# SandraLouise/SVJedi-graph

Measured on AMD Instinct MI355X. Metric: GAF alignments classified/sec (classify + count all-reduce + genotype, text resident in HBM), higher is better.
Workload: dtype u8/int64 (classify), f64 (likelihood)

## Files before the change

svjedi-graph_amd/csrc/svjg_capi.hip:

```cpp
#include "svjg_kernels.h"
#include "svjg_host_tables.h"
#include "svjg_pass.h"
#include <rccl/rccl.h>
#include <errno.h>
#include <math.h>
#include <stdio.h>
#include <stdlib.h>
#include <string.h>
#include <fcntl.h>
#include <unistd.h>
#include <string>
#include <thread>
#include <vector>

using namespace svjg;
typedef struct svjg_ctx svjg_ctx;

static thread_local std::string g_init_error;

#include <memory>
#include <mutex>
namespace {
struct TablesCache {
    std::mutex mu;
// ... 18 lines not shown
    h = fold64(g.chrom_names, (size_t)g.chrom_off[g.n_chrom], h);
    const uint64_t tail[3] = {g.d_over, g.flags, g.n_slots};
    return fold64(tail, sizeof tail, h);
}

std::shared_ptr<const KernelTables> kernel_tables_for(const svjg_graph &g) {
    const uint64_t key[6] = {g.n_nodes, g.n_edges, g.n_hits, g.n_chrom, graph_digest(g, 1), graph_digest(g, 0xD6E8FEB86659FD93ull)};
    std::lock_guard<std::mutex> lk(g_tables.mu);
    if (!g_tables.kt || memcmp(key, g_tables.key, sizeof key) != 0) {
        g_tables.kt = std::make_shared<const KernelTables>(build_kernel_tables(g));
        memcpy(g_tables.key, key, sizeof key);
    }
    return g_tables.kt;
}
}

extern "C" void svjg_release_host_tables(void) {
    std::lock_guard<std::mutex> lk(g_tables.mu);
    g_tables.kt.reset();
    memset(g_tables.key, 0, sizeof g_tables.key);
}

constexpr int STAGE_THREADS = 4;
constexpr uint64_t STAGE_PIECE = 8ull << 20;

constexpr int RUN_SLOTS = 3;

struct svjg_ctx {
    int device = 0;
    int wall_khz = 0;
    int n_cu = 256;
    int occ_main = 0;
    hipStream_t stream = nullptr, copy_stream = nullptr;
    hipEvent_t ev[6] = {};
    std::string err;
    bool have_graph = false, have_counts = false;
    svjg_node *d_nodes = nullptr;  svjg_edge *d_edges = nullptr;  uint32_t *d_hits = nullptr;
    uint8_t *d_cnames = nullptr;   uint32_t *d_coff = nullptr, *d_clo = nullptr, *d_chash = nullptr, *d_names = nullptr, *d_links = nullptr, *d_nok = nullptr;  uint16_t *d_disp = nullptr;  uint32_t *d_ihits = nullptr, *d_pfx = nullptr;
    GraphView gv{};
    uint32_t names_len = 0, gflags = 0, n_slots = 0;
    unsigned long long *d_counts = nullptr, *d_snap = nullptr;
    uint8_t *d_gaf = nullptr;  uint64_t gaf_cap = 0, gaf_bytes = 0;  bool have_gaf = false;
    char *h_stage[STAGE_THREADS * 2] = {};
    hipStream_t stage_stream[STAGE_THREADS] = {};
    hipEvent_t stage_ev[STAGE_THREADS * 2] = {};
    uint64_t *d_deferred = nullptr;  uint64_t deferred_cap = 0;
    svjg_hitrec *d_recs = nullptr;   uint64_t rec_cap = 0;
    uint64_t *d_host = nullptr;      uint64_t host_cap = 0;
    DevStatus *d_st = nullptr;
    unsigned long long *d_dbg = nullptr;
    uint32_t *d_long = nullptr;
    DevStatus *h_stp = nullptr;
    DevStatus &hs() { return *h_stp; }
    uint64_t total_deferred = 0;
    dd *d_logfact = nullptr;  uint32_t logfact_n = 0;  dd *d_bsum = nullptr;
    unsigned int *d_maxn = nullptr;
    void *d_rows = nullptr;  uint64_t rows_cap = 0;
    void *h_rows = nullptr;  uint64_t h_rows_cap = 0;
    uint64_t geno_rows = 0;
    struct RunSlot {
        void *d = nullptr;  uint64_t d_cap = 0;  void *h = nullptr;  uint64_t h_cap = 0;  void *h_dev = nullptr;
        unsigned long long *counts = nullptr;  uint64_t counts_cap = 0;
        hipEvent_t ev[6] = {};  hipEvent_t computed = nullptr, copied = nullptr;
        uint64_t base_offset = 0;  uint32_t min_support = 0;  double err = 0;  bool had_text = false, slow_end_own = false, timed_by_events = false;
        bool clean = false;
    } run[RUN_SLOTS];
    int run_head = 0, run_tail = 0, run_inflight = 0;
    int counts_in_slot = -1;
    void *d_run_in = nullptr;  uint64_t d_run_in_cap = 0;  uint64_t run_rows = 0;  bool have_rows = false;
    float ms_main = 0, ms_slow = 0, ms_geno = 0;
    float ms_main_stamps = 0, ms_main_events = 0;
    ncclComm_t comm = nullptr;
    bool allreduce_second = false;
    uint64_t part_total = 0, part_need = 0, part_next = 0;
};

#define HIPCHK(ctx, call)                                                                         \
    do {                                                                                          \
        hipError_t e_ = (call);                                                                   \
        if (e_ != hipSuccess) {                                                                   \
            (ctx)->err = std::string(#call) + ": " + hipGetErrorString(e_);                       \
            return SVJG_E_HIP;                                                                    \
        }                                                                                         \
    } while (0)

extern "C" int svjg_abi_version(void) { return SVJG_ABI_VERSION; }

extern "C" int svjg_device_count(void) {
    int n = 0;
    if (hipGetDeviceCount(&n) != hipSuccess) return 0;
    return n;
}

extern "C" const char *svjg_last_error(const svjg_ctx *ctx) { return ctx ? ctx->err.c_str() : g_init_error.c_str(); }

extern "C" int svjg_init(int device, svjg_ctx **out) {
    if (!out) return SVJG_E_ARG;
    *out = nullptr;
    int n = 0;
    hipError_t e = hipGetDeviceCount(&n);
    if (e != hipSuccess || n <= 0) {
        g_init_error = "no HIP device visible (libsvjg_hip has no CPU fallback)";
        return SVJG_E_NO_DEVICE;
    }
    if (device < 0 || device >= n) { g_init_error = "device index out of range"; return SVJG_E_ARG; }
    svjg_ctx *c = new svjg_ctx();
// ... 21 lines not shown
}

static void free_graph(svjg_ctx *c) {
    hipFree(c->d_nodes); hipFree(c->d_edges); hipFree(c->d_hits); hipFree(c->d_cnames); hipFree(c->d_coff);
    hipFree(c->d_clo); hipFree(c->d_chash); hipFree(c->d_counts); hipFree(c->d_snap); hipFree(c->d_names); hipFree(c->d_links); hipFree(c->d_disp); hipFree(c->d_ihits); hipFree(c->d_nok); hipFree(c->d_pfx);
    c->d_pfx = nullptr; c->d_nok = nullptr; c->d_names = nullptr; c->d_links = nullptr; c->d_disp = nullptr; c->d_ihits = nullptr;
    c->d_nodes = nullptr; c->d_edges = nullptr; c->d_hits = nullptr; c->d_cnames = nullptr; c->d_coff = nullptr;
    c->d_clo = nullptr; c->d_chash = nullptr; c->d_counts = nullptr; c->d_snap = nullptr;
    c->have_graph = false; c->have_counts = false;
    for (auto &r : c->run) r.clean = false;
}

extern "C" void svjg_destroy(svjg_ctx *c) {
    if (!c) return;
    hipSetDevice(c->device);
    if (c->stream) hipStreamSynchronize(c->stream);
    if (c->copy_stream) hipStreamSynchronize(c->copy_stream);
    if (c->comm) ncclCommDestroy(c->comm);
    free_graph(c);
    hipFree(c->d_long);
    hipFree(c->d_gaf); hipFree(c->d_deferred); hipFree(c->d_recs); hipFree(c->d_host); hipFree(c->d_st); hipFree(c->d_logfact);
    hipFree(c->d_bsum); hipFree(c->d_maxn); hipFree(c->d_rows); hipFree(c->d_run_in);
    for (auto &r : c->run) {
        hipFree(r.d); hipFree(r.counts);
        if (r.h) hipHostFree(r.h);
        for (auto &e : r.ev) if (e) hipEventDestroy(e);
        if (r.computed) hipEventDestroy(r.computed);
        if (r.copied) hipEventDestroy(r.copied);
    }
    if (c->h_rows) hipHostFree(c->h_rows);
    if (c->h_stp) hipHostFree(c->h_stp);
    for (auto &b : c->h_stage) if (b) hipHostFree(b);
    for (auto &ev : c->stage_ev) if (ev) hipEventDestroy(ev);
    for (auto &st : c->stage_stream) if (st) hipStreamDestroy(st);
    for (auto &ev : c->ev) if (ev) hipEventDestroy(ev);
    if (c->copy_stream) hipStreamDestroy(c->copy_stream);
    if (c->stream) hipStreamDestroy(c->stream);
    delete c;
}

template <class T>
static int upload(svjg_ctx *c, T **dst, const T *src, uint64_t n, uint64_t extra = 0) {
    HIPCHK(c, hipMalloc((void **)dst, (n + extra + 1) * sizeof(T)));
    if (n) HIPCHK(c, hipMemcpyAsync(*dst, src, n * sizeof(T), hipMemcpyHostToDevice, c->stream));
    return 0;
}

#ifndef SVJG_SMALL_CHUNK
#define SVJG_SMALL_CHUNK 65536
#endif
#ifndef SVJG_FIRST_SHARE
#define SVJG_FIRST_SHARE 0.85
#endif
constexpr uint64_t SMALL_CHUNK = SVJG_SMALL_CHUNK;
constexpr double FIRST_CHUNK_SHARE = SVJG_FIRST_SHARE;

static int reset_status(svjg_ctx *c, bool all) {
    if (all) {
        c->hs() = c->h_stp[1]; c->total_deferred = 0;
        HIPCHK(c, hipMemcpyAsync(c->d_st, &c->h_stp[1], sizeof(DevStatus), hipMemcpyHostToDevice, c->stream));
        return 0;
    }
    c->hs().n_deferred = 0; c->hs().overflow = 0; c->hs().next_chunk = 0;
    HIPCHK(c, hipMemcpyAsync(c->d_st, &c->hs(), sizeof(DevStatus), hipMemcpyHostToDevice, c->stream));
    return 0;
}

extern "C" int svjg_load_graph(svjg_ctx *c, const svjg_graph *g) {
    if (!c || !g || !g->nodes || !g->chrom_off || !g->chrom_node_lo) return SVJG_E_ARG;
    if (g->n_nodes >= 0x7FFFFFFFull || g->n_edges >= 0x7FFFFFFFull || g->n_chrom >= 65535) { c->err = "graph too large"; return SVJG_E_ARG; }
    if (g->d_over >= 0x80000000u) { c->err = "d_over too large"; return SVJG_E_ARG; }
    HIPCHK(c, hipSetDevice(c->device));
    free_graph(c);
    int rc;
    struct Undo { svjg_ctx *c; bool armed = true; ~Undo() { if (armed) { hipStreamSynchronize(c->stream); free_graph(c); } } } undo{c};
    if ((rc = upload(c, &c->d_nodes, g->nodes, g->n_nodes + 1))) return rc;
    if ((rc = upload(c, &c->d_edges, g->edges, g->n_edges))) return rc;
    if ((rc = upload(c, &c->d_hits, g->hits, g->n_hits))) return rc;
    c->names_len = g->chrom_off[g->n_chrom];
    if ((rc = upload(c, &c->d_cnames, (const uint8_t *)g->chrom_names, c->names_len, 8))) return rc;
    if ((rc = upload(c, &c->d_coff, g->chrom_off, g->n_chrom + 1))) return rc;
    if ((rc = upload(c, &c->d_clo, g->chrom_node_lo, g->n_chrom + 1))) return rc;
    std::vector<uint32_t> hash = build_chrom_hash(*g);
    if ((rc = upload(c, &c->d_chash, hash.data(), hash.size()))) return rc;
    const std::shared_ptr<const KernelTables> ktp = kernel_tables_for(*g);
    const KernelTables &kt = *ktp;
    if ((rc = upload(c, &c->d_names, kt.names.data(), kt.names.size()))) return rc;
    if ((rc = upload(c, &c->d_links, kt.links.data(), kt.links.size()))) return rc;
    if ((rc = upload(c, &c->d_disp, kt.disp.data(), kt.disp.size()))) return rc;
    if ((rc = upload(c, &c->d_ihits, kt.ihits.data(), kt.ihits.size()))) return rc;
    if ((rc = upload(c, &c->d_nok, kt.node_of_kid.data(), kt.node_of_kid.size()))) return rc;
    if (!kt.name_pfx.empty() && (rc = upload(c, &c->d_pfx, kt.name_pfx.data(), kt.name_pfx.size()))) return rc;
    HIPCHK(c, hipStreamSynchronize(c->stream));
    c->gv.nodes = c->d_nodes; c->gv.n_nodes = (uint32_t)g->n_nodes; c->gv.edges = c->d_edges; c->gv.hits = c->d_hits;
    c->gv.chrom_names = c->d_cnames; c->gv.chrom_off = c->d_coff; c->gv.chrom_lo = c->d_clo; c->gv.chrom_hash = c->d_chash;
    c->gv.n_chrom = g->n_chrom; c->gv.hash_mask = (uint32_t)hash.size() - 1; c->gv.d_over = g->d_over;
    c->gv.dover_list = (g->flags & SVJG_GRAPH_DOVER_LIST) ? 1u : 0u;
    c->gv.name_pfx = c->d_pfx;
    c->gv.node_of_kid = c->d_nok; c->gv.name_tab = c->d_names; c->gv.name_ihits = c->d_ihits; c->gv.name_disp = c->d_disp; c->gv.name_slots = kt.name_slots; c->gv.name_buckets = kt.name_buckets;
    c->gv.name_complete = (kt.names_left_out == 0 && kt.names_skipped == 0) ? 1u : 0u;
    c->gv.link_tab = c->d_links; c->gv.link_mask = kt.link_mask; c->gv.link_seed = kt.link_seed;
    c->gflags = g->flags;
    if (g->flags & SVJG_GRAPH_DOVER_LIST) c->gflags |= SVJG_GRAPH_ALL_SLOW;
    if (kt.links_left_out) c->gflags |= SVJG_GRAPH_ALL_SLOW;
    c->n_slots = g->n_slots;
    HIPCHK(c, hipMalloc((void **)&c->d_counts, ((uint64_t)g->n_slots + GUARD_WORDS) * 8));
    HIPCHK(c, hipMalloc((void **)&c->d_snap, ((uint64_t)g->n_slots + GUARD_WORDS) * 8));
    c->have_graph = true; c->have_counts = true;
    undo.armed = false;
    return svjg_reset_counts(c);
}

extern "C" int svjg_alloc_counts(svjg_ctx *c, uint32_t n_slots) {
    if (!c) return SVJG_E_ARG;
    HIPCHK(c, hipSetDevice(c->device));
    free_graph(c);
// ... 116 lines not shown
        if (rc) return rc;
    }
    return gaf_finish(c, n, need);
}

static int ensure(svjg_ctx *c, void **p, uint64_t *cap, uint64_t want, size_t elem, bool keep) {
    if (want <= *cap) return 0;
    const uint64_t asked = want;
    if (keep && *cap && want < *cap + *cap / 2) want = *cap + *cap / 2;
    void *q = nullptr;
    if (want != asked && hipMalloc(&q, want * elem) != hipSuccess) { (void)hipGetLastError(); q = nullptr; want = asked; }
    if (!q) HIPCHK(c, hipMalloc(&q, want * elem));
    if (keep && *p && *cap) HIPCHK(c, hipMemcpyAsync(q, *p, *cap * elem, hipMemcpyDeviceToDevice, c->stream));
    HIPCHK(c, hipStreamSynchronize(c->stream));
    hipFree(*p);
    *p = q; *cap = want;
    return 0;
}

static int fetch_slot_counts(svjg_ctx *c) {
    if (c->counts_in_slot < 0) return 0;
    const int k = c->counts_in_slot;
    c->counts_in_slot = -1;
    HIPCHK(c, hipSetDevice(c->device));
    if (c->run[k].copied) HIPCHK(c, hipStreamWaitEvent(c->stream, c->run[k].copied, 0));
    HIPCHK(c, hipMemcpyAsync(c->d_counts, c->run[k].counts, ((uint64_t)c->n_slots + GUARD_WORDS) * 8, hipMemcpyDeviceToDevice, c->stream));
    return 0;
}

static uint64_t deferred_want(const svjg_ctx *c, uint64_t n) { return (c->gflags & SVJG_GRAPH_ALL_SLOW) ? n / 24 + 64 : (n / 4096 + 65536); }

static void main_launch_setup(svjg_ctx *c, uint64_t begin, uint64_t end, uint64_t base_offset, int want_hits, ClassifyArgs &a, uint32_t &grid, size_t &lds) {
    const uint64_t n = end - begin;
    const bool all_slow = (c->gflags & SVJG_GRAPH_ALL_SLOW) != 0;
    a.gaf = c->d_gaf; a.begin = begin; a.n_bytes = end; a.base_offset = base_offset; a.g = c->gv;
    a.all_slow = all_slow; a.want_hits = want_hits != 0;
#ifdef SVJG_ABLATE
    { const char *dg = getenv("SVJG_DIAG"); a.diag = dg ? (uint32_t)atoi(dg) : 0u; }
#endif
    a.counts = c->d_counts; a.deferred = c->d_deferred; a.deferred_cap = c->deferred_cap;
    a.recs = c->d_recs; a.rec_cap = c->rec_cap; a.host_lines = c->d_host; a.host_cap = c->host_cap; a.st = c->d_st; a.dbg = c->d_dbg;
    lds = LDS_MAIN;
    if (c->occ_main < 1) {
        int occ = 0;
        if (hipOccupancyMaxActiveBlocksPerMultiprocessor(&occ, k_classify_main, (int)WG, lds) != hipSuccess || occ < 1) occ = 1;
        const int by_lds = (int)((160u * 1024u) / ((lds + LDS_GRANULE - 1) / LDS_GRANULE * LDS_GRANULE));
        if (by_lds >= 1 && occ > by_lds) occ = by_lds;
        c->occ_main = occ;
        hipFree(c->d_long); c->d_long = nullptr;
#ifdef SVJG_ABLATE
        { const char *oc = getenv("SVJG_OCC"); fprintf(stderr, "[svjg diag] occupancy API: %d workgroups of %u threads per CU (LDS %zu)\n", occ, WG, lds); if (oc && atoi(oc) > 0) c->occ_main = atoi(oc); }
#endif
    }
    const uint64_t full = (uint64_t)c->n_cu * (uint64_t)c->occ_main;
    if (!c->d_long && hipMalloc((void **)&c->d_long, full * LONG_WORDS * sizeof(uint32_t)) != hipSuccess) c->d_long = nullptr;
    a.long_pre = c->d_long;
    const uint64_t share = (n + full - 1) / full;
    uint64_t region = (share + 15) & ~15ull;
    a.small = 0;
    if (share >= 8 * SMALL_CHUNK) { region = ((uint64_t)(share * FIRST_CHUNK_SHARE) + 15) & ~15ull; a.small = SMALL_CHUNK; }
    if (region < TEXT) region = TEXT;
    a.region = region;
    const uint64_t want_grid = (n + region - 1) / region;
    grid = (uint32_t)(want_grid < full ? want_grid : full);
}

constexpr uint64_t EXACT_ROUND_PER_CU = 4;
constexpr uint64_t STEP_WAVE_ROUNDS = 30;
constexpr uint64_t FUSED_WAVE_ROUNDS = 16;
static int launch_exact(svjg_ctx *c, const ClassifyArgs &a, uint64_t wave_rounds, const NextPass &nx) {
    const uint64_t wave_limit = wave_rounds * EXACT_ROUND_PER_CU * (uint64_t)c->n_cu;
    hipLaunchKernelGGL(k_classify_exact, dim3((uint32_t)c->n_cu * EXACT_BLOCKS_PER_CU), dim3(EXACT_TPB), 0, c->stream, a, wave_limit, nx);
    HIPCHK(c, hipGetLastError());
    return 0;
}

static int classify_range(svjg_ctx *c, uint64_t begin, uint64_t end, uint64_t base_offset, int want_hits) {
    HIPCHK(c, hipSetDevice(c->device));
    { const int rc0 = fetch_slot_counts(c); if (rc0) return rc0; }
    if (end <= begin) return 0;
    const uint64_t n = end - begin;
    uint64_t def_want = deferred_want(c, n);
    uint64_t rec_want = want_hits ? c->hs().n_recs + n / 40 + 65536 : 0;
    uint64_t host_want = c->hs().n_host + 4096;
    int rc;
    for (int attempt = 0; attempt < 3; ++attempt) {
        if ((rc = ensure(c, (void **)&c->d_deferred, &c->deferred_cap, def_want, sizeof(uint64_t), false))) return rc;
        if ((rc = ensure(c, (void **)&c->d_host, &c->host_cap, host_want, sizeof(uint64_t), true))) return rc;
        if (want_hits && (rc = ensure(c, (void **)&c->d_recs, &c->rec_cap, rec_want, sizeof(svjg_hitrec), true))) return rc;
        HIPCHK(c, hipMemcpyAsync(c->d_snap, c->d_counts, ((uint64_t)c->n_slots + GUARD_WORDS) * 8, hipMemcpyDeviceToDevice, c->stream));
        DevStatus before = c->hs();
        if ((rc = reset_status(c, false))) return rc;
        ClassifyArgs a{};
        uint32_t grid = 0;
        size_t lds = 0;
        main_launch_setup(c, begin, end, base_offset, want_hits, a, grid, lds);
        if (!a.long_pre) { c->err = "no memory for the workers' scratch words"; return SVJG_E_NOMEM; }
#ifdef SVJG_TIMING
        if (a.diag & 16u) HIPCHK(c, hipMemsetAsync(c->d_dbg, 0, 32 * 8, c->stream));
#endif
        HIPCHK(c, hipEventRecord(c->ev[0], c->stream));
        hipLaunchKernelGGL(k_classify_main, dim3(grid), dim3(WG), lds, c->stream, a);
        HIPCHK(c, hipGetLastError());
        HIPCHK(c, hipEventRecord(c->ev[1], c->stream));
        HIPCHK(c, hipMemcpyAsync(&c->hs(), c->d_st, sizeof(DevStatus), hipMemcpyDeviceToHost, c->stream));
        HIPCHK(c, hipStreamSynchronize(c->stream));
        const uint64_t n_def = c->hs().n_deferred;
#ifdef SVJG_TIMING
        if (a.diag & 16u) {
            unsigned long long d[16];
            HIPCHK(c, hipMemcpy(d, c->d_dbg, sizeof d, hipMemcpyDeviceToHost));
            fprintf(stderr, "[svjg diag] sub-passes of long lines: first sweep counting %llu, first sweep measuring only %llu, second sweep %llu; nodes in sub-passes %llu\n", d[12], d[13], d[14], d[15]);
            fprintf(stderr, "[svjg diag] wave time per phase (sum over waves, counter ticks)  A+B1 %llu  prefix %llu  B2 %llu  R1 %llu  NP: lists %llu  names+disp %llu  records %llu  scan+search %llu  links+atomics %llu  R6+end %llu;  passes %llu (sub-passes of long lines %llu), nodes in them %llu\n",
                    d[0], d[1], d[2], d[3], d[8], d[9], d[4], 0ull, d[6], d[7], d[10], d[11], d[5]);
        }
#endif
        c->ms_slow = 0;
        if (n_def && !(c->hs().overflow & 1u)) {
            HIPCHK(c, hipEventRecord(c->ev[2], c->stream));
            if ((rc = launch_exact(c, a, STEP_WAVE_ROUNDS, NextPass{}))) return rc;
            HIPCHK(c, hipEventRecord(c->ev[3], c->stream));
            HIPCHK(c, hipMemcpyAsync(&c->hs(), c->d_st, sizeof(DevStatus), hipMemcpyDeviceToHost, c->stream));
            HIPCHK(c, hipStreamSynchronize(c->stream));
            HIPCHK(c, hipEventElapsedTime(&c->ms_slow, c->ev[2], c->ev[3]));
#ifdef SVJG_TIMING
            if (a.diag & 16u) {
                unsigned long long d[8];
                HIPCHK(c, hipMemcpy(d, c->d_dbg + 16, sizeof d, hipMemcpyDeviceToHost));
                fprintf(stderr, "[svjg diag] one wave per line, the longest any line took per step (counter ticks): terminator + staging %llu  per-line part %llu  piece table %llu  nodes %llu  links %llu\n",
                        d[0], d[1], d[2], d[3], d[4]);
                unsigned long long l[5];
                HIPCHK(c, hipMemcpy(l, c->d_dbg + 24, sizeof l, hipMemcpyDeviceToHost));
                fprintf(stderr, "[svjg diag] one lane per line, ticks summed over the blocks of 64 lines: terminators + staging %llu  per-line part %llu  nodes %llu  links %llu  rest %llu\n",
                        l[0], l[1], l[2], l[3], l[4]);
            }
#endif
        }
        HIPCHK(c, hipEventElapsedTime(&c->ms_main, c->ev[0], c->ev[1]));
        if (!c->hs().overflow) {
            c->total_deferred += n_def;
            break;
        }
        if (attempt == 2) { c->err = "output buffers overflowed repeatedly"; return SVJG_E_NOMEM; }
        if (c->hs().overflow & 1u) def_want = n / 24 + 64;
        if (c->hs().overflow & 2u) rec_want = before.n_recs + (c->hs().n_recs - before.n_recs) * 2 + n / 24 + 64;
        if (c->hs().overflow & 4u) host_want = before.n_host + n / 24 + 64;
        HIPCHK(c, hipMemcpyAsync(c->d_counts, c->d_snap, ((uint64_t)c->n_slots + GUARD_WORDS) * 8, hipMemcpyDeviceToDevice, c->stream));
        uint64_t keep_err = before.err;
        c->hs() = before; c->hs().err = keep_err;
    }
    if (c->hs().err != ~0ull) return SVJG_E_INPUT;
    return 0;
}

extern "C" int svjg_classify_resident(svjg_ctx *c, uint64_t base_offset, int want_hits) {
    if (!c || !c->have_graph || !c->have_gaf) { if (c) c->err = "classify needs a graph and an uploaded GAF"; return SVJG_E_ARG; }
    return classify_range(c, 0, c->gaf_bytes, base_offset, want_hits);
}

constexpr uint64_t PIPE_BYTES = 128ull << 20;
// ... 655 lines not shown
```

svjedi-graph_amd/csrc/svjg_kernels.h:

```cpp
#pragma once
#include <hip/hip_runtime.h>
#define SVJG_TAB_AS __attribute__((address_space(3)))
#include "svjg_line.h"
#include "svjg_planes.h"
#include "svjg_pass.h"
#include "svjg_geno.h"

namespace svjg {

constexpr uint32_t WG = 64;
constexpr uint32_t TPB = 256;
constexpr uint32_t PIECES = 4;
constexpr uint32_t SPAN = PIECES * 16;
constexpr uint32_t HALF = SPAN * WG;
constexpr uint32_t NHALF = 2;
constexpr uint32_t TEXT = NHALF * HALF;
constexpr uint32_t MAXL = 64;
#ifndef SVJG_CAP_O
#ifdef SVJG_W16
#define SVJG_CAP_O 208
#else
#define SVJG_CAP_O 216
#endif
#endif
constexpr uint32_t CAP_O = SVJG_CAP_O;
constexpr uint32_t KMAX = 64;
#ifdef SVJG_W16
constexpr uint32_t KLONG = KMAX;
#else
constexpr uint32_t KLONG = CAP_O < 255u ? CAP_O : 255u;
#endif
constexpr uint32_t LONG_LOG = 256;
constexpr uint32_t LONG_WORDS = 3 * LONG_LOG;
static_assert(KLONG <= LONG_LOG && KLONG * 4 <= TEXT / 8 + 16, "a long line's per-node words fit their places");
constexpr uint32_t LRW = MAXL;
static_assert(TEXT + 1 < 65535, "text offsets are kept in 16 bits, 0xFFFF = none");

constexpr uint32_t L_TEXT = 0;
#ifdef SVJG_W16
constexpr uint32_t L_TBM = L_TEXT + TEXT + 64;
constexpr uint32_t L_NDBM = L_TBM;
constexpr uint32_t L_RL = L_TBM;
constexpr uint32_t L_OPL = L_TBM + TEXT / 8 + 16;
constexpr uint32_t L_LINE = L_OPL + (CAP_O + 8) * 3;
constexpr uint32_t LDS_MAIN = L_LINE + (MAXL + 8) * 4;
constexpr uint32_t LDS_GRANULE = 1280;
static_assert(LDS_MAIN <= 8 * LDS_GRANULE, "sixteen workers per CU");
static_assert(L_TBM % 16 == 0 && L_OPL % 16 == 0 && L_LINE % 4 == 0, "LDS alignment");
#else
constexpr uint32_t L_NDBM = L_TEXT + TEXT + 64;
constexpr uint32_t L_RL = L_NDBM;
constexpr uint32_t L_TBM = L_NDBM + TEXT / 8 + 16;
constexpr uint32_t L_OPL = L_TBM + TEXT / 8 + 16;
constexpr uint32_t L_LINE = L_OPL + (CAP_O + 8) * 4;
constexpr uint32_t LDS_MAIN = L_LINE + (MAXL + 8) * 4;
constexpr uint32_t LDS_GRANULE = 1280;
static_assert(LRW * 16 <= TEXT / 8 + 16, "the per-line records fit the bitmap they replace");
static_assert(LDS_MAIN <= 9 * LDS_GRANULE, "fourteen workers per CU");
static_assert(L_NDBM % 16 == 0 && L_TBM % 16 == 0 && L_OPL % 16 == 0 && L_LINE % 16 == 0 && L_RL % 16 == 0, "LDS alignment");
#endif

struct DevStatus {
    unsigned long long n_lines;
    unsigned long long n_deferred;
    unsigned long long n_recs;
    unsigned long long err;
    unsigned int non_ascii;
    unsigned int overflow;
    unsigned long long next_chunk;
    unsigned long long n_host;
    unsigned long long cause[8];
    unsigned long long t_first, t_last;
    unsigned long long t_exact;
};

struct ClassifyArgs {
    const uint8_t *gaf;
    uint64_t begin;
    uint64_t n_bytes;
    uint64_t base_offset;
    GraphView g;
    uint32_t all_slow;
    uint32_t want_hits;
    uint64_t region;
    uint64_t small;
    uint32_t diag;
    unsigned long long *counts;
    uint64_t *deferred;  uint64_t deferred_cap;
    svjg_hitrec *recs;   uint64_t rec_cap;
    uint64_t *host_lines; uint64_t host_cap;
    DevStatus *st;
    unsigned long long *dbg;
    uint32_t *long_pre;
};

__device__ inline uint32_t zero_bytes(uint32_t t) {
    return ~(((t & 0x7F7F7F7Fu) + 0x7F7F7F7Fu) | t | 0x7F7F7F7Fu);
}
__device__ inline uint32_t eq_mask16(uint4 v, uint32_t pat) {
    const uint32_t lo = __builtin_amdgcn_udot4(zero_bytes(v.x ^ pat), 0x08040201u, __builtin_amdgcn_udot4(zero_bytes(v.y ^ pat), 0x80402010u, 0u, false), false);
    const uint32_t hi = __builtin_amdgcn_udot4(zero_bytes(v.z ^ pat), 0x08040201u, __builtin_amdgcn_udot4(zero_bytes(v.w ^ pat), 0x80402010u, 0u, false), false);
    return (lo | (hi << 8)) >> 7;
}

__device__ inline uint32_t wave_incl_scan(uint32_t v) {
    uint32_t x = v;
    asm("s_nop 1\n\tv_add_u32_dpp %0, %0, %0 row_shr:1 row_mask:0xf bank_mask:0xf bound_ctrl:0\n\t"
        "s_nop 1\n\tv_add_u32_dpp %0, %0, %0 row_shr:2 row_mask:0xf bank_mask:0xf bound_ctrl:0\n\t"
        "s_nop 1\n\tv_add_u32_dpp %0, %0, %0 row_shr:4 row_mask:0xf bank_mask:0xf bound_ctrl:0\n\t"
        "s_nop 1\n\tv_add_u32_dpp %0, %0, %0 row_shr:8 row_mask:0xf bank_mask:0xf bound_ctrl:0\n\t"
        "s_nop 1\n\tv_add_u32_dpp %0, %0, %0 row_bcast:15 row_mask:0xa bank_mask:0xf\n\t"
        "s_nop 1\n\tv_add_u32_dpp %0, %0, %0 row_bcast:31 row_mask:0xc bank_mask:0xf"
        : "+v"(x));
    return x;
}
__device__ inline void wave_incl_scan2(uint32_t &x, uint32_t &y) {
#define SVJG_STEP(ctl) "s_nop 0\n\tv_add_u32_dpp %0, %0, %0 " ctl "\n\tv_add_u32_dpp %1, %1, %1 " ctl "\n\t"
    asm("s_nop 0\n\t"
        SVJG_STEP("row_shr:1 row_mask:0xf bank_mask:0xf bound_ctrl:0") SVJG_STEP("row_shr:2 row_mask:0xf bank_mask:0xf bound_ctrl:0")
        SVJG_STEP("row_shr:4 row_mask:0xf bank_mask:0xf bound_ctrl:0") SVJG_STEP("row_shr:8 row_mask:0xf bank_mask:0xf bound_ctrl:0")
        SVJG_STEP("row_bcast:15 row_mask:0xa bank_mask:0xf") SVJG_STEP("row_bcast:31 row_mask:0xc bank_mask:0xf")
        : "+v"(x), "+v"(y));
#undef SVJG_STEP
}
__device__ inline unsigned long long ballot64(bool p) { return __builtin_amdgcn_ballot_w64(p); }
typedef unsigned long long wmask;
#define RARELY(c) __builtin_expect((c) != 0, 0)
__device__ inline wmask m_eq(uint32_t a, uint32_t b) { return __builtin_amdgcn_uicmp(a, b, 32); }
__device__ inline wmask m_ne(uint32_t a, uint32_t b) { return __builtin_amdgcn_uicmp(a, b, 33); }
__device__ inline wmask m_gt(uint32_t a, uint32_t b) { return __builtin_amdgcn_uicmp(a, b, 34); }
__device__ inline wmask m_ge(uint32_t a, uint32_t b) { return __builtin_amdgcn_uicmp(a, b, 35); }
__device__ inline wmask m_lt(uint32_t a, uint32_t b) { return __builtin_amdgcn_uicmp(a, b, 36); }
__device__ inline wmask m_le(uint32_t a, uint32_t b) { return __builtin_amdgcn_uicmp(a, b, 37); }
__device__ inline bool in_mask(wmask m) { return __builtin_amdgcn_inverse_ballot_w64(m); }
__device__ inline uint32_t rdlane(uint32_t v, uint32_t l) { return (uint32_t)__builtin_amdgcn_readlane((int)v, (int)l); }
__device__ inline uint32_t lane_below_or(uint32_t v, uint32_t first) { return (uint32_t)__builtin_amdgcn_update_dpp((int)first, (int)v, 0x138, 0xF, 0xF, false); }
__device__ inline uint32_t lane_below(uint32_t v) { return (uint32_t)__builtin_amdgcn_update_dpp((int)v, (int)v, 0x138, 0xF, 0xF, false); }
__device__ inline uint32_t lane_above(uint32_t v) { return (uint32_t)__builtin_amdgcn_update_dpp((int)v, (int)v, 0x130, 0xF, 0xF, false); }
// ... 237 lines not shown
    uint8_t *text = lds + L_TEXT;
    uint32_t *ndbm = (uint32_t *)(lds + L_NDBM);
    uint32_t *tbm = (uint32_t *)(lds + L_TBM);
#ifdef SVJG_W16
    uint16_t *OPLP = (uint16_t *)(lds + L_OPL);
    uint8_t *OPLL = lds + L_OPL + (CAP_O + 8) * 2;
#define OPL_PUT(j, v) do { const uint32_t v_ = (v); OPLP[j] = (uint16_t)v_; OPLL[j] = (uint8_t)((v_ >> 16) + 1u); } while (0)
#define OPL_POS(j) ((uint32_t)OPLP[j])
#else
    uint32_t *OPL = (uint32_t *)(lds + L_OPL);
#define OPL_PUT(j, v) OPL[j] = (v)
#define OPL_POS(j) (OPL[j] & 0xFFFFu)
#endif
    uint32_t *LINE = (uint32_t *)(lds + L_LINE);
    uint4 *RL = (uint4 *)(lds + L_RL);

    const uint32_t lane = threadIdx.x;
    const GraphView g = a.g;

    unsigned long long pos = a.begin + (unsigned long long)blockIdx.x * a.region;
    if (blockIdx.x == 0 && lane == 0) a.st->t_first = wall_clock64();
    if (pos >= a.n_bytes) return;
    unsigned long long rend = pos + a.region < a.n_bytes ? pos + a.region : a.n_bytes;

    if (lane < 4) tbm[TEXT / 32 + lane] = 0;
    unsigned long long wave_lines = 0;
#ifdef SVJG_TIMING
    unsigned long long stamp = __builtin_readcyclecounter(), acc[16] = {0, 0, 0, 0, 0, 0, 0, 0, 0, 0, 0, 0, 0, 0, 0, 0};
    auto tick = [&](int ph) { const unsigned long long t = __builtin_readcyclecounter(); acc[ph] += t - stamp; stamp = t; };
#define tick_mem(ph) do { asm volatile("s_waitcnt vmcnt(0) lgkmcnt(0)" ::: "memory"); tick(ph); } while (0)
#define tally(ph, n) do { acc[ph] += (n); } while (0)
#elif defined(SVJG_MARK)
#define tick(ph) asm volatile("; MARK " #ph)
#else
    auto tick = [](int) {};
#endif
#ifndef SVJG_TIMING
#define tick_mem(ph) do { } while (0)
#define tally(ph, n) do { } while (0)
#endif

    constexpr uint32_t NPF = HALF / (WG * 16);
    uint4 pf[NPF];
    uint32_t pf_head = '\n';
    typedef uint32_t u32x4 __attribute__((ext_vector_type(4)));
    auto fetch_half = [&](unsigned long long at) {
        const uint4 *src = (const uint4 *)(a.gaf + at) + lane;
#pragma unroll
        for (uint32_t i = 0; i < NPF; ++i) {
            const u32x4 v = __builtin_nontemporal_load((const u32x4 *)(src + i * WG));
            pf[i] = make_uint4(v.x, v.y, v.z, v.w);
        }
    };
  for (;;) {
    fetch_half(pos & ~15ull);
    { const unsigned long long c0 = pos & ~15ull; pf_head = c0 > a.begin ? a.gaf[c0 - 1] : (uint32_t)'\n'; }

    for (;;) {
        const unsigned long long c0 = pos & ~15ull;
        const uint32_t own_lo = (uint32_t)(pos - c0);
        const uint32_t V = (uint32_t)((a.n_bytes - c0 < (unsigned long long)TEXT) ? (a.n_bytes - c0) : (unsigned long long)TEXT);
        const bool at_eof = c0 + V == a.n_bytes;

        const uint32_t head_byte = pf_head;
        unsigned long long NL[NHALF], ORI[NHALF];
        SpanFlags fl = {0u, 0u, 0u, 0u};
        uint32_t dee_end = 0;
        unsigned long long IDM[NHALF];
#pragma unroll
        for (uint32_t h = 0; h < NHALF; ++h) {
            __builtin_amdgcn_s_setprio(P_A);
#pragma unroll
            for (uint32_t i = 0; i < NPF; ++i) *(uint4 *)(text + h * HALF + (i * WG + lane) * 16) = pf[i];
            if (h + 1 < NHALF) fetch_half(c0 + (h + 1) * HALF);
            wave_sync();
            __builtin_amdgcn_s_setprio(0);
            fl.idf = 0u;
            classify_span(a, text, ndbm, tbm, h, h * WG + lane, c0, V, NL[h], ORI[h], fl);
            IDM[h] = ballot64(fl.idf != 0);
            if (h == 0) dee_end = rdlane(fl.dee_last, WG - 1);
            else if (dee_end != 0 && text[HALF] == ':') {
                IDM[0] |= 1ull << 63;
                if (lane == WG - 1) { const uint32_t c = (fl.idsum >> 6) & 3u; fl.idsum = (fl.idsum & 0xFF00u) | ((c < 3u ? c + 1u : 3u) << 6) | 63u; }
            }
        }
        if (ballot64(fl.high != 0) != 0 && lane == 0) a.st->non_ascii = 1;
        const bool idf = (IDM[0] | IDM[1]) != 0;
        if (idf && lane == 0) {
            LINE[MAXL + 4] = (uint32_t)IDM[0]; LINE[MAXL + 5] = (uint32_t)(IDM[0] >> 32); LINE[MAXL + 6] = (uint32_t)IDM[1]; LINE[MAXL + 7] = (uint32_t)(IDM[1] >> 32);
        }
        tick(0);
        const uint32_t head = (head_byte == '\n') || (head_byte == '\r' && text[0] != '\n');
        uint32_t Vh = V;
        bool eof_h = at_eof;
        uint32_t lim2, n_s, n_own, tot_ori, l_first;
        bool last_stripe, long_line;
        unsigned long long next_pos;
        uint32_t RK[NHALF];
        uint32_t head_own;
        for (uint32_t attempt = 0;; ++attempt) {
            uint32_t s_last = NONE32;
            {
                const unsigned long long b1 = ballot64(NL[1] != 0), b0 = ballot64(NL[0] != 0);
                if (b1 | b0) {
                    const uint32_t hh = b1 ? 1u : 0u;
                    const uint32_t L = 63u - (uint32_t)__builtin_clzll(b1 ? b1 : b0);
                    const uint32_t mlo = (uint32_t)__builtin_amdgcn_readlane((int)(uint32_t)(hh ? NL[1] : NL[0]), (int)L);
                    const uint32_t mhi = (uint32_t)__builtin_amdgcn_readlane((int)(uint32_t)((hh ? NL[1] : NL[0]) >> 32), (int)L);
                    const unsigned long long m = ((unsigned long long)mhi << 32) | mlo;
                    s_last = (hh * WG + L) * SPAN + (63u - (uint32_t)__builtin_clzll(m)) + 1u;
                } else if (head) s_last = 0;
            }
            const uint32_t own_lim = rend - c0 < (unsigned long long)Vh ? (uint32_t)(rend - c0) : Vh;
            lim2 = own_lim;
            last_stripe = false; long_line = false;
            next_pos = c0 + Vh;
            if (eof_h) last_stripe = true;
// ... 38 lines not shown
            uint32_t cut = 0;
            {
                const unsigned long long f1 = ballot64(best[1] != 0), f0 = ballot64(best[0] != 0);
                if (f1) cut = rdlane(best[1], 63u - (uint32_t)__builtin_clzll(f1));
                else if (f0) cut = rdlane(best[0], 63u - (uint32_t)__builtin_clzll(f0));
            }
            if (cut > own_lo && cut > 16u) Vh = cut;
            else if (Vh > HALF) Vh = HALF;
            else break;
            eof_h = false;
#pragma unroll
            for (uint32_t h = 0; h < NHALF; ++h) {
                const unsigned long long keep = low_bits64(clamp64(Vh, (h * WG + lane) * SPAN));
                NL[h] &= keep; ORI[h] &= keep;
            }
        }
        if (RARELY(long_line) && Vh == TEXT && !a.all_slow && tot_ori <= CAP_O && text[TEXT - 1] != 'd') {
            unsigned long long at = c0 + TEXT, E = ~0ull;
            bool clean = true;
            for (uint32_t it = 0; it < 64u && clean && E == ~0ull; ++it, at += HALF) {
                if (at >= a.n_bytes) { E = a.n_bytes; break; }
                fetch_half(at);
#pragma unroll
                for (uint32_t i = 0; i < NPF; ++i) {
                    if (E != ~0ull || !clean) break;
                    const uint4 v = pf[i];
                    const uint32_t nl = eq_mask16(v, 0x0A0A0A0Au), dee = eq_mask16(v, 0x64646464u), col = eq_mask16(v, 0x3A3A3A3Au);
                    const uint32_t bad = eq_mask16(v, 0x0D0D0D0Du) | (dee & ((col >> 1) | 0x8000u));
                    if (ballot64(((v.x | v.y | v.z | v.w) & 0x80808080u) != 0) != 0 && lane == 0) a.st->non_ascii = 1;
                    uint32_t front = 0xFFFFu;
                    const unsigned long long b = ballot64(nl != 0);
                    if (b != 0) {
                        const uint32_t L = (uint32_t)__builtin_ctzll(b), bit = (uint32_t)__builtin_ctz(rdlane(nl, L));
                        E = at + (unsigned long long)((i * WG + L) * 16u + bit);
                        front = lane < L ? 0xFFFFu : lane == L ? (1u << bit) - 1u : 0u;
                    }
                    if (ballot64((bad & front) != 0) != 0) clean = false;
                }
                if (E != ~0ull && E >= a.n_bytes) E = a.n_bytes;
            }
            if (clean && E != ~0ull) {
                eof_h = true;
                next_pos = E < a.n_bytes ? E + 1ull : a.n_bytes;
                last_stripe = next_pos >= rend;
            }
        }
        if (!last_stripe) {
            if (RARELY(long_line && eof_h)) pf_head = (next_pos & 15ull) ? (uint32_t)'x' : (uint32_t)'\n';
            else {
                const uint32_t d0 = (uint32_t)((next_pos & ~15ull) - c0);
                pf_head = d0 ? (uint32_t)text[d0 - 1] : head_byte;
            }
            fetch_half(next_pos & ~15ull);
        }
        tick(1);

        if (a.all_slow || (long_line && !eof_h) || n_s > MAXL || tot_ori > CAP_O) {
            if (n_own) {
                unsigned long long dbase = 0;
                if (lane == 0) { dbase = atomicAdd(&a.st->n_deferred, (unsigned long long)n_own); atomicAdd(&a.st->cause[DC_STRIPE], (unsigned long long)n_own); }
                dbase = __shfl(dbase, 0);
                if (lane == 0 && head_own) { if (dbase < a.deferred_cap) a.deferred[dbase] = c0; else atomicOr(&a.st->overflow, 1u); }
#pragma unroll
                for (uint32_t h = 0; h < NHALF; ++h) {
                    const uint32_t sp = (h * WG + lane) * SPAN;
                    uint32_t j = (RK[h] & 0xFFFFu) + ((h == 0 && lane == 0) ? head : 0u) - l_first;
                    for (unsigned long long m = NL[h]; m; m &= m - 1, ++j) {
                        if (j >= n_own) continue;
                        const unsigned long long d = dbase + j;
                        if (d < a.deferred_cap) a.deferred[d] = c0 + sp + (uint32_t)__builtin_ctzll(m) + 1u; else atomicOr(&a.st->overflow, 1u);
                    }
                }
            }
            wave_lines += n_own;
            wave_sync();
            if (last_stripe) break;
            pos = next_pos;
            continue;
        }

        if (DIAG(32u)) { wave_lines += n_own; if (last_stripe) break; pos = next_pos; continue; }
        __builtin_amdgcn_s_setprio(P_B2);
        if (lane == 0) {
            if (head) LINE[0] = 0u;
            LINE[n_s] = 0xFFFFu | (tot_ori << 16);
        }
#pragma unroll
        for (uint32_t h = 0; h < NHALF; ++h) {
            const uint32_t sp = (h * WG + lane) * SPAN;
            const uint32_t sb = (RK[h] & 0xFFFFu) + ((h == 0 && lane == 0) ? head : 0u);
            const uint32_t ob = RK[h] >> 16;
            uint32_t j = sb;
            for (unsigned long long m = NL[h]; m; m &= m - 1, ++j) {
                const uint32_t b = (uint32_t)__builtin_ctzll(m);
                LINE[j] = (sp + b + 1) | ((ob + (uint32_t)__popcll(ORI[h] & ((1ull << b) - 1ull))) << 16);
            }
            j = ob;
            if (ballot64((NL[h] & (NL[h] - 1ull)) != 0) == 0) {
                const uint32_t t1 = NL[h] ? (uint32_t)__builtin_ctzll(NL[h]) : 64u;
                const uint32_t v0 = sp + ((sb - 1u) << 16);
                for (unsigned long long m = ORI[h]; m; m &= m - 1, ++j) {
                    const uint32_t b = (uint32_t)__builtin_ctzll(m);
                    OPL_PUT(j, v0 + b + (b > t1 ? 0x10000u : 0u));
                }
            } else {
                for (unsigned long long m = ORI[h]; m; m &= m - 1, ++j) {
// ... 464 lines not shown
                    if (fb >= upto) break;
                    if (fb == 0u) long_words_sync();
                    const uint32_t *LG = a.long_pre + (size_t)blockIdx.x * LONG_WORDS + LONG_LOG + 2u * (fb + lane_c);
                    nh = 0; hp = nullptr;
                    if (fb + lane_c < upto) {
                        const uint32_t w0 = __hip_atomic_load(LG, __ATOMIC_RELAXED, __HIP_MEMORY_SCOPE_WORKGROUP);
                        const uint32_t w1 = __hip_atomic_load(LG + 1, __ATOMIC_RELAXED, __HIP_MEMORY_SCOPE_WORKGROUP);
                        if (w0 != 0xFFFFFFFFu) {
                            if (w1 & 0x80000000u) { hp = ((w1 & 0x40000000u) ? g.name_ihits : g.hits) + w0; nh = (w1 & 0x3FFFFFFFu) | 0x80000000u; }
                            else { h0 = w0; h1 = w1; nh = w1 == 0x7FFFFFFFu ? 1u : 2u; }
                        }
                    }
                    __builtin_amdgcn_s_waitcnt(0x0F70);
                    fb += WG;
                }
                tick(6);
                if (RARELY(lsub) && (lsub & L_FINAL)) { ++i0; lsub = 0; }
            }
#undef lD0
#undef lP
#undef lR
#undef SET_D0
#undef SET_P
#undef SET_R
            wave_sync();
            {
                const uint32_t fin = RL[lane].z >> 24;
                const bool defer = lane < cnt && fin >= ST_DEFER;
                unsigned long long db = ballot64(defer);
                if (RARELY(db)) {
#pragma unroll
                    for (uint32_t cse = 0; cse < DC_STRIPE; ++cse) {
                        const unsigned long long cb = ballot64(defer && fin == ST_DEFER + cse);
                        if (cb && lane == 0) atomicAdd(&a.st->cause[cse], (unsigned long long)__popcll(cb));
                    }
                    unsigned long long dbase = 0;
                    if (lane == 0) dbase = atomicAdd(&a.st->n_deferred, (unsigned long long)__popcll(db));
                    dbase = __shfl(dbase, 0);
                    if (defer) {
                        unsigned long long idx = dbase + __popcll(db & ((1ull << lane) - 1ull));
                        if (idx < a.deferred_cap) a.deferred[idx] = c0 + s; else atomicOr(&a.st->overflow, 1u);
                    }
                }
            }
            wave_sync();
            __builtin_amdgcn_s_setprio(P_R1);
        }
        wave_lines += n_own;
        wave_sync();
        tick(7);
        if (last_stripe) break;
        pos = next_pos;
    }
    if (!a.small) break;
    unsigned long long ci = 0;
    if (lane == 0) ci = atomicAdd(&a.st->next_chunk, 1ull);
    ci = ((unsigned long long)(uint32_t)__builtin_amdgcn_readfirstlane((int)(uint32_t)(ci >> 32)) << 32) | (uint32_t)__builtin_amdgcn_readfirstlane((int)(uint32_t)ci);
    pos = a.begin + (unsigned long long)gridDim.x * a.region + ci * a.small;
    if (pos >= a.n_bytes) break;
    rend = pos + a.small < a.n_bytes ? pos + a.small : a.n_bytes;
  }
    if (lane == 0 && wave_lines) atomicAdd(&a.st->n_lines, wave_lines);
    if (lane == 0) atomicMax(&a.st->t_last, (unsigned long long)wall_clock64());
#ifdef SVJG_TIMING
    if ((a.diag & 16u) && lane == 0)
        for (int i = 0; i < 16; ++i) atomicAdd(&a.dbg[i], acc[i]);
#endif
}

typedef uint32_t svjg_u32x4 __attribute__((ext_vector_type(4)));
__global__ __launch_bounds__(TPB) void k_copy16(uint4 *dst, const uint4 *src, uint64_t n16) {
    const uint64_t stride = (uint64_t)gridDim.x * TPB;
    uint64_t i = (uint64_t)blockIdx.x * TPB + threadIdx.x;
    for (; i + 3 * stride < n16; i += 4 * stride) {
        const svjg_u32x4 a = __builtin_nontemporal_load((const svjg_u32x4 *)(src + i)), b = __builtin_nontemporal_load((const svjg_u32x4 *)(src + i + stride));
        const svjg_u32x4 c = __builtin_nontemporal_load((const svjg_u32x4 *)(src + i + 2 * stride)), d = __builtin_nontemporal_load((const svjg_u32x4 *)(src + i + 3 * stride));
        __builtin_nontemporal_store(a, (svjg_u32x4 *)(dst + i)); __builtin_nontemporal_store(b, (svjg_u32x4 *)(dst + i + stride));
        __builtin_nontemporal_store(c, (svjg_u32x4 *)(dst + i + 2 * stride)); __builtin_nontemporal_store(d, (svjg_u32x4 *)(dst + i + 3 * stride));
    }
    for (; i < n16; i += stride) dst[i] = src[i];
}
__global__ __launch_bounds__(TPB) void k_read16(uint4 *sink, const uint4 *src, uint64_t n16) {
    const uint64_t stride = (uint64_t)gridDim.x * TPB;
    uint64_t i = (uint64_t)blockIdx.x * TPB + threadIdx.x;
    uint32_t acc = 0;
    for (; i + 3 * stride < n16; i += 4 * stride) {
        const svjg_u32x4 a = __builtin_nontemporal_load((const svjg_u32x4 *)(src + i)), b = __builtin_nontemporal_load((const svjg_u32x4 *)(src + i + stride));
        const svjg_u32x4 c = __builtin_nontemporal_load((const svjg_u32x4 *)(src + i + 2 * stride)), d = __builtin_nontemporal_load((const svjg_u32x4 *)(src + i + 3 * stride));
        acc ^= a.x ^ a.w ^ b.y ^ b.z ^ c.x ^ c.w ^ d.y ^ d.z;
    }
    for (; i < n16; i += stride) acc ^= src[i].x;
    if (acc == 0x12345677u) sink[0].x = acc;
}

struct NextPass { unsigned long long *counts; uint64_t n_words; DevStatus *st; unsigned int *max_n; };
__device__ __forceinline__ void reset_next_pass(const NextPass &nx, uint64_t first, uint64_t stride) {
    for (uint64_t i = first; i < nx.n_words; i += stride) nx.counts[i] = 0ull;
    if (first == 0) {
        DevStatus z{}; z.err = ~0ull;
        *nx.st = z;
        nx.max_n[0] = 0u; nx.max_n[1] = 0u;
    }
}
__global__ __launch_bounds__(TPB) void k_step_reset(NextPass nx) {
    reset_next_pass(nx, (uint64_t)blockIdx.x * TPB + threadIdx.x, (uint64_t)gridDim.x * TPB);
}

__device__ inline void report_line(const ClassifyArgs &a, unsigned long long off, int rc) {
    if (rc == SVJG_EXC_ASK_HOST) {
        const unsigned long long i = atomicAdd(&a.st->n_host, 1ull);
        if (i < a.host_cap) a.host_lines[i] = off; else atomicOr(&a.st->overflow, 4u);
    } else atomicMin(&a.st->err, (off << 3) | (unsigned long long)rc);
}

struct SlowEmit {
    const ClassifyArgs *a;
// ... 440 lines not shown
```

Measured before the change: 8.103 billion.

## Prefetch next dynamic chunk during last stripe and add configurable tail geometry

The dynamic chunk claim now happens while the final stripe of the current range is still being processed, so the next chunk's first text block (including the preceding byte) is prefetched before the stripe finishes instead of after. Chunk geometry becomes env-configurable, with separately sized tail chunks near the end of the input meant to shrink end-of-kernel drain. Per-worker end timestamps are accumulated so the drain can be reported. This adds two extra atomics per wave and a 32-bit chunk counter, and the head-byte staging logic gets more complex.

Result: slower. 7.718 billion (-4.8%).

```diff
diff --git a/svjedi-graph_amd/csrc/svjg_capi.hip b/svjedi-graph_amd/csrc/svjg_capi.hip
--- a/svjedi-graph_amd/csrc/svjg_capi.hip
+++ b/svjedi-graph_amd/csrc/svjg_capi.hip
@@ -94,6 +94,7 @@
     uint32_t *d_long = nullptr;
     DevStatus *h_stp = nullptr;
     DevStatus &hs() { return *h_stp; }
+    bool geo_report = false;
     uint64_t total_deferred = 0;
     dd *d_logfact = nullptr;  uint32_t logfact_n = 0;  dd *d_bsum = nullptr;
     unsigned int *d_maxn = nullptr;
@@ -221,8 +222,46 @@
 #ifndef SVJG_FIRST_SHARE
 #define SVJG_FIRST_SHARE 0.85
 #endif
+#ifndef SVJG_TAIL_CHUNK
+#define SVJG_TAIL_CHUNK SVJG_SMALL_CHUNK
+#endif
+#ifndef SVJG_TAIL_PER_WORKER
+#define SVJG_TAIL_PER_WORKER 2
+#endif
 constexpr uint64_t SMALL_CHUNK = SVJG_SMALL_CHUNK;
 constexpr double FIRST_CHUNK_SHARE = SVJG_FIRST_SHARE;
+constexpr uint64_t TAIL_CHUNK = SVJG_TAIL_CHUNK;
+constexpr uint64_t TAIL_PER_WORKER = SVJG_TAIL_PER_WORKER;
+
+struct Geometry {
+    bool cut = false, report = false;
+    uint64_t workers = 0, chunk = SMALL_CHUNK, tail = TAIL_CHUNK, tail_per_worker = TAIL_PER_WORKER;
+    int64_t tail_from = -1;
+    double first = FIRST_CHUNK_SHARE;
+};
+static Geometry geometry_from_env() {
+    Geometry g;
+    const char *e = getenv("SVJG_GEOMETRY");
+    if (!e) return g;
+    auto bytes16 = [](const char *v) -> uint64_t { const uint64_t b = strtoull(v, nullptr, 10) & ~15ull; return b < 64 ? 64 : b > (1ull << 30) ? (1ull << 30) : b; };
+    for (const char *p = e; *p;) {
+        const char *q = strchr(p, ','); const size_t len = q ? (size_t)(q - p) : strlen(p);
+        const std::string kv(p, len);
+        const size_t eq = kv.find('=');
+        if (eq != std::string::npos) {
+            const std::string k = kv.substr(0, eq); const char *v = kv.c_str() + eq + 1;
+            if (k == "workers") { g.workers = strtoull(v, nullptr, 10); g.cut = true; }
+            else if (k == "first") { g.first = atof(v); if (!(g.first > 0.0)) g.first = 0.01; if (g.first > 1.0) g.first = 1.0; g.cut = true; }
+            else if (k == "chunk") { g.chunk = bytes16(v); g.cut = true; }
+            else if (k == "tail") { g.tail = bytes16(v); g.cut = true; }
+            else if (k == "tail_from") { g.tail_from = (int64_t)strtoull(v, nullptr, 10); g.cut = true; }
+            else if (k == "tail_per_worker") g.tail_per_worker = strtoull(v, nullptr, 10);
+            else if (k == "report") g.report = atoi(v) != 0;
+        }
+        p += len; if (*p == ',') ++p;
+    }
+    return g;
+}
 
 static int reset_status(svjg_ctx *c, bool all) {
     if (all) {
@@ -230,7 +269,7 @@
         HIPCHK(c, hipMemcpyAsync(c->d_st, &c->h_stp[1], sizeof(DevStatus), hipMemcpyHostToDevice, c->stream));
         return 0;
     }
-    c->hs().n_deferred = 0; c->hs().overflow = 0; c->hs().next_chunk = 0;
+    c->hs().n_deferred = 0; c->hs().overflow = 0; c->hs().next_chunk = 0; c->hs().t_end_sum = 0; c->hs().n_ended = 0;
     HIPCHK(c, hipMemcpyAsync(c->d_st, &c->hs(), sizeof(DevStatus), hipMemcpyHostToDevice, c->stream));
     return 0;
 }
@@ -453,17 +492,27 @@
         { const char *oc = getenv("SVJG_OCC"); fprintf(stderr, "[svjg diag] occupancy API: %d workgroups of %u threads per CU (LDS %zu)\n", occ, WG, lds); if (oc && atoi(oc) > 0) c->occ_main = atoi(oc); }
 #endif
     }
-    const uint64_t full = (uint64_t)c->n_cu * (uint64_t)c->occ_main;
-    if (!c->d_long && hipMalloc((void **)&c->d_long, full * LONG_WORDS * sizeof(uint32_t)) != hipSuccess) c->d_long = nullptr;
+    const Geometry geo = geometry_from_env();
+    const uint64_t slots = (uint64_t)c->n_cu * (uint64_t)c->occ_main;
+    const uint64_t full = geo.workers && geo.workers < slots ? geo.workers : slots;
+    if (!c->d_long && hipMalloc((void **)&c->d_long, slots * LONG_WORDS * sizeof(uint32_t)) != hipSuccess) c->d_long = nullptr;
     a.long_pre = c->d_long;
     const uint64_t share = (n + full - 1) / full;
     uint64_t region = (share + 15) & ~15ull;
-    a.small = 0;
-    if (share >= 8 * SMALL_CHUNK) { region = ((uint64_t)(share * FIRST_CHUNK_SHARE) + 15) & ~15ull; a.small = SMALL_CHUNK; }
+    a.small = 0; a.tail = 0; a.tail_from = 0;
+    if (geo.cut || share >= 8 * SMALL_CHUNK) { region = ((uint64_t)(share * geo.first) + 15) & ~15ull; a.small = geo.chunk; }
     if (region < TEXT) region = TEXT;
     a.region = region;
     const uint64_t want_grid = (n + region - 1) / region;
     grid = (uint32_t)(want_grid < full ? want_grid : full);
+    if (a.small) {
+        const uint64_t fixed = (uint64_t)grid * region, dyn = n > fixed ? n - fixed : 0;
+        const uint64_t tail_bytes = geo.tail_per_worker * (uint64_t)grid * geo.tail;
+        uint64_t from = geo.tail_from >= 0 ? (uint64_t)geo.tail_from : dyn > tail_bytes ? (dyn - tail_bytes) / a.small : 0;
+        if (from > 0xFFFFFFFEull) from = 0xFFFFFFFEull;
+        a.tail = (uint32_t)geo.tail; a.tail_from = (uint32_t)from;
+    }
+    c->geo_report = geo.report;
 }
 
 constexpr uint64_t EXACT_ROUND_PER_CU = 4;
@@ -507,6 +556,13 @@
         HIPCHK(c, hipMemcpyAsync(&c->hs(), c->d_st, sizeof(DevStatus), hipMemcpyDeviceToHost, c->stream));
         HIPCHK(c, hipStreamSynchronize(c->stream));
         const uint64_t n_def = c->hs().n_deferred;
+        if (c->geo_report) {
+            const DevStatus &t = c->hs();
+            const double us = c->wall_khz ? 1e3 / (double)c->wall_khz : 0.0, span = (double)(t.t_last - t.t_first) * us;
+            const double mean_end = t.n_ended ? (double)(t.t_end_sum - t.n_ended * t.t_first) / (double)t.n_ended * us : 0.0;
+            fprintf(stderr, "[svjg geometry] grid %u region %llu chunk %llu tail %u from chunk %u; claims %llu; launch %.1f us, mean worker end %.1f us, drain %.1f us (%.2f %%)\n",
+                    grid, (unsigned long long)a.region, (unsigned long long)a.small, a.tail, a.tail_from, (unsigned long long)(uint32_t)t.next_chunk, span, mean_end, span - mean_end, span > 0 ? 100.0 * (span - mean_end) / span : 0.0);
+        }
 #ifdef SVJG_TIMING
         if (a.diag & 16u) {
             unsigned long long d[16];
diff --git a/svjedi-graph_amd/csrc/svjg_kernels.h b/svjedi-graph_amd/csrc/svjg_kernels.h
--- a/svjedi-graph_amd/csrc/svjg_kernels.h
+++ b/svjedi-graph_amd/csrc/svjg_kernels.h
@@ -72,6 +72,8 @@
     unsigned long long cause[8];
     unsigned long long t_first, t_last;
     unsigned long long t_exact;
+    unsigned long long t_end_sum;
+    unsigned long long n_ended;
 };
 
 struct ClassifyArgs {
@@ -84,6 +86,8 @@
     uint32_t want_hits;
     uint64_t region;
     uint64_t small;
+    uint32_t tail_from;
+    uint32_t tail;
     uint32_t diag;
     unsigned long long *counts;
     uint64_t *deferred;  uint64_t deferred_cap;
@@ -427,17 +431,22 @@
             pf[i] = make_uint4(v.x, v.y, v.z, v.w);
         }
     };
+    constexpr uint32_t STAGED_BACK = 0x100u;
+    uint32_t claim = NONE32;
+    const unsigned long long dyn0 = a.begin + (unsigned long long)gridDim.x * a.region;
+    auto chunk_at = [&](uint32_t ci) -> unsigned long long {
+        return ci < a.tail_from ? dyn0 + (unsigned long long)ci * a.small : dyn0 + (unsigned long long)a.tail_from * a.small + (unsigned long long)(ci - a.tail_from) * a.tail;
+    };
+    if (pos > a.begin) { fetch_half((pos - 1ull) & ~15ull); pf_head = (uint32_t)'x' | STAGED_BACK; }
+    else fetch_half(pos & ~15ull);
   for (;;) {
-    fetch_half(pos & ~15ull);
-    { const unsigned long long c0 = pos & ~15ull; pf_head = c0 > a.begin ? a.gaf[c0 - 1] : (uint32_t)'\n'; }
-
     for (;;) {
-        const unsigned long long c0 = pos & ~15ull;
+        const unsigned long long c0 = (pos - (unsigned long long)(pf_head >> 8)) & ~15ull;
         const uint32_t own_lo = (uint32_t)(pos - c0);
         const uint32_t V = (uint32_t)((a.n_bytes - c0 < (unsigned long long)TEXT) ? (a.n_bytes - c0) : (unsigned long long)TEXT);
         const bool at_eof = c0 + V == a.n_bytes;
 
-        const uint32_t head_byte = pf_head;
+        const uint32_t head_byte = pf_head & 0xFFu;
         unsigned long long NL[NHALF], ORI[NHALF];
         SpanFlags fl = {0u, 0u, 0u, 0u};
         uint32_t dee_end = 0;
@@ -582,6 +591,12 @@
                 pf_head = d0 ? (uint32_t)text[d0 - 1] : head_byte;
             }
             fetch_half(next_pos & ~15ull);
+        } else if (a.small) {
+            uint32_t ci = 0;
+            if (lane == 0) ci = atomicAdd((unsigned int *)&a.st->next_chunk, 1u);
+            ci = (uint32_t)__builtin_amdgcn_readfirstlane((int)ci);
+            const unsigned long long at = chunk_at(ci);
+            if (at < a.n_bytes) { claim = ci; pf_head = (uint32_t)'x' | STAGED_BACK; fetch_half((at - 1ull) & ~15ull); }
         }
         tick(1);
 
@@ -1152,16 +1167,18 @@
         if (last_stripe) break;
         pos = next_pos;
     }
-    if (!a.small) break;
-    unsigned long long ci = 0;
-    if (lane == 0) ci = atomicAdd(&a.st->next_chunk, 1ull);
-    ci = ((unsigned long long)(uint32_t)__builtin_amdgcn_readfirstlane((int)(uint32_t)(ci >> 32)) << 32) | (uint32_t)__builtin_amdgcn_readfirstlane((int)(uint32_t)ci);
-    pos = a.begin + (unsigned long long)gridDim.x * a.region + ci * a.small;
-    if (pos >= a.n_bytes) break;
-    rend = pos + a.small < a.n_bytes ? pos + a.small : a.n_bytes;
+    if (claim == NONE32) break;
+    pos = chunk_at(claim);
+    { const unsigned long long sz = claim < a.tail_from ? a.small : (unsigned long long)a.tail; rend = pos + sz < a.n_bytes ? pos + sz : a.n_bytes; }
+    claim = NONE32;
   }
     if (lane == 0 && wave_lines) atomicAdd(&a.st->n_lines, wave_lines);
-    if (lane == 0) atomicMax(&a.st->t_last, (unsigned long long)wall_clock64());
+    if (lane == 0) {
+        const unsigned long long t_end = wall_clock64();
+        atomicMax(&a.st->t_last, t_end);
+        atomicAdd(&a.st->t_end_sum, t_end);
+        atomicAdd(&a.st->n_ended, 1ull);
+    }
 #ifdef SVJG_TIMING
     if ((a.diag & 16u) && lane == 0)
         for (int i = 0; i < 16; ++i) atomicAdd(&a.dbg[i], acc[i]);
```
